# Bhumbra/probayes

Hardware: AMD Instinct MI355X
Metric: MH chain-steps/sec (whole node), 10-dim model, 65 536 chains, 1/2/4/8 GPU (higher is better)
Workload: dtype f64; 1 GPU; cfg2: 10-dim diagonal-Gaussian random-walk MH, 65536 chains/GPU, full trace every step; chains_per_gpu=65536, dim=10, trace=True, steps_per_launch=250, parallelism=chain-sharded x1

## Files before the change

probayes_amd/csrc/pbh_device.h:

```cpp
#pragma once
#include <hip/hip_runtime.h>
#include <stdint.h>

namespace pbh {

constexpr double kNearlyPosZero = 2.2250738585072014e-308;
constexpr double kNearlyPosInf = 1.7976931348623158e+308;
constexpr double kNearlyNegInf = -1.7976931348623158e+308;


struct u32x4 { uint32_t x, y, z, w; };

__device__ __forceinline__ u32x4 philox4x32_10(u32x4 c, uint32_t k0,
                                                uint32_t k1) {
  constexpr uint32_t M0 = 0xD2511F53u, M1 = 0xCD9E8D57u;
  constexpr uint32_t W0 = 0x9E3779B9u, W1 = 0xBB67AE85u;
#pragma unroll
  for (int i = 0; i < 10; ++i) {
    const uint64_t p0 = (uint64_t)M0 * c.x;
    const uint64_t p1 = (uint64_t)M1 * c.z;
    const uint32_t hi0 = (uint32_t)(p0 >> 32), lo0 = (uint32_t)p0;
    const uint32_t hi1 = (uint32_t)(p1 >> 32), lo1 = (uint32_t)p1;
    c = u32x4{(uint32_t)__builtin_amdgcn_bitop3_b32(hi1, c.y, k0, 0x96), lo1,
              (uint32_t)__builtin_amdgcn_bitop3_b32(hi0, c.w, k1, 0x96), lo0};
    k0 += W0;
    k1 += W1;
  }
  return c;
}

struct PhiloxKeys { uint32_t k0[10], k1[10]; };
__device__ __forceinline__ uint32_t in_vgpr(uint32_t v) {
  uint32_t r;
  asm("v_mov_b32 %0, %1" : "=v"(r) : "s"(v));
  return r;
}
__device__ __forceinline__ double in_vgpr_f64(double v) {
  const uint64_t b = __builtin_bit_cast(uint64_t, v);
  return __builtin_bit_cast(double, ((uint64_t)in_vgpr((uint32_t)(b >> 32)) << 32) |
                                        in_vgpr((uint32_t)b));
}
__device__ __forceinline__ PhiloxKeys philox_keys_v(uint32_t k0, uint32_t k1) {
  PhiloxKeys k;
#pragma unroll
  for (int i = 0; i < 10; ++i) {
    k.k0[i] = in_vgpr(k0 + (uint32_t)i * 0x9E3779B9u);
    k.k1[i] = in_vgpr(k1 + (uint32_t)i * 0xBB67AE85u);
  }
  return k;
}
__device__ __forceinline__ u32x4 philox4x32_10_rk(u32x4 c, const PhiloxKeys &k) {
  constexpr uint32_t M0 = 0xD2511F53u, M1 = 0xCD9E8D57u;
#pragma unroll
  for (int i = 0; i < 10; ++i) {
    const uint64_t p0 = (uint64_t)M0 * c.x;
    const uint64_t p1 = (uint64_t)M1 * c.z;
    const uint32_t hi0 = (uint32_t)(p0 >> 32), lo0 = (uint32_t)p0;
    const uint32_t hi1 = (uint32_t)(p1 >> 32), lo1 = (uint32_t)p1;
    c = u32x4{(uint32_t)__builtin_amdgcn_bitop3_b32(hi1, c.y, k.k0[i], 0x96), lo1,
              (uint32_t)__builtin_amdgcn_bitop3_b32(hi0, c.w, k.k1[i], 0x96), lo0};
  }
  return c;
}

struct Xo { uint32_t s0, s1, s2, s3; };

__device__ __forceinline__ uint32_t rotl32(uint32_t x, int k) {
  return (x << k) | (x >> (32 - k));
}

__device__ __forceinline__ uint32_t xo_next(Xo &s) {
  const uint32_t r = rotl32(s.s1 * 5u, 7) * 9u;
  const uint32_t t = s.s1 << 9;
  s.s2 ^= s.s0;
  s.s3 ^= s.s1;
  s.s1 ^= s.s2;
  s.s0 ^= s.s3;
  s.s2 ^= t;
  s.s3 = rotl32(s.s3, 11);
  return r;
}

__host__ __device__ __forceinline__ uint64_t splitmix64(uint64_t &z) {
  uint64_t x = (z += 0x9E3779B97F4A7C15ull);
  x = (x ^ (x >> 30)) * 0xBF58476D1CE4E5B9ull;
  x = (x ^ (x >> 27)) * 0x94D049BB133111EBull;
  return x ^ (x >> 31);
}

__device__ __forceinline__ double u01(uint32_t a, uint32_t b) {
  return ((double)(a >> 5) * 67108864.0 + (double)(b >> 6)) *
         (1.0 / 9007199254740992.0);
}

__device__ __forceinline__ void box_muller(u32x4 w, double &z0, double &z1) {
  const double u1 = 1.0 - u01(w.x, w.y);
  const double u2 = u01(w.z, w.w);
  const double r = sqrt(-2.0 * log(u1));
  double s, c;
  sincospi(2.0 * u2, &s, &c);
  z0 = r * c;
  z1 = r * s;
}

__device__ __forceinline__ double log_unit(double u) {
  const uint64_t b = __builtin_bit_cast(uint64_t, u);
  int e = (int)((b >> 52) & 0x7FF) - 1023;
  double m = __builtin_bit_cast(double, (b & 0x000FFFFFFFFFFFFFull) |
                                            0x3FF0000000000000ull);
  const bool big = m > 1.4142135623730951;
  m = big ? m * 0.5 : m;
  e += big ? 1 : 0;
  const double t = (m - 1.0) / (m + 1.0);
  const double s = t * t;
// ... 644 lines not shown
```

probayes_amd/csrc/pbh_engine.hip:

```cpp
#include <hip/hip_runtime.h>
#include <rccl/rccl.h>

#include <cmath>
#include <cstdarg>
#include <cstdio>
#include <cstdlib>
#include <cstring>
#include <string>
#include <algorithm>
#include <atomic>
#include <chrono>
#include <map>
#include <mutex>
#include <unordered_map>
#include <vector>

#include "../../include/pbhip.h"
#include "pbh_kernels.h"
#include "pbh_expr_host.h"
#include "pbh_device.h"

using pbh::KArgs;

struct pbh_engine {
// ... 1331 lines not shown
      return fail(PBH_ERR_STATE, "trace capacity %lld < %lld records",
                  (long long)e->cap, (long long)recs);
  }
  return PBH_OK;
}

static void run_args(pbh_engine *e, KArgs &k, size_t &lds) {
  k = e->k;
  k.n = e->n;
  k.off = e->off;
  k.x = e->x;
  k.lp = e->lp;
  k.rng = e->rng;
  k.seed_lo = (uint32_t)e->seed;
  k.seed_hi = (uint32_t)(e->seed >> 32);
  k.rep = e->rep;
#ifdef PBH_PHASES
  if (!k.rep) k.rep = phase_buffer();
#endif
  k.xo = e->xo;
  k.tx = e->tx; k.tlp = e->tlp; k.tpx = e->tpx; k.tpp = e->tpp; k.ts = e->ts;
  k.tacc = e->tacc;
  k.thin = e->cap > 0 ? e->thin : 1;
  k.rec_base = e->rec_base;
  k.rec_cap = e->cap;
  k.debug = e->debug;
  k.W = (e->n + 63) / 64;
  {
    const double v = k.tran_value;
    const double qt = k.pscale == PBH_PSCALE_LIN
                          ? v : (v <= k.log_npi ? std::exp(v) : 1.7976931348623158e+308);
    k.pair_ok = (e->pair_enabled && (k.scores == PBH_SCORES_METROPOLIS || qt > 0.0)) ? 1 : 0;
    k.simple_acc = (k.scores == PBH_SCORES_METROPOLIS ||
                    (k.scores == PBH_SCORES_HASTINGS &&
                     k.tran_kind == PBH_TRAN_CONST && qt > 0.0)) ? 1 : 0;
    k.acc_beta = (k.scores == PBH_SCORES_HASTINGS && !k.tran_sym) ? qt : 1.0;
  }
  k.gibbs_mfma = e->gibbs_mfma ? 1 : 0;
  k.gibbs_fast = e->gibbs_fast ? 1 : 0;
  k.gibbs_lanes = e->gibbs_lanes;
  k.gmm_lanes = e->gmm_lanes;
  k.gmm_full = e->gmm_full ? 1 : 0;
  k.pair_full = e->pair_full ? 1 : 0;
  k.iid_full = e->iid_full ? 1 : 0;
  k.fair = e->fair;
  k.pair_wg = e->pair_wg;
  k.gq = e->gq;
  k.moments = (e->collect & PBH_COLLECT_MOMENTS) ? 1 : 0;
  k.msum = e->msum; k.msq = e->msq; k.nacc = e->nacc;
  k.bm64 = e->bm64;
  lds = (k.target == PBH_TARGET_NORM_IID && k.tn <= 16384 &&
                      k.rng != PBH_RNG_PHILOX)
                         ? (size_t)k.tn * sizeof(double) : 0;
}

int pbh_run(pbh_engine *e, int64_t n_steps, int32_t steps_per_launch) {
  if (check_ptr(e, "engine")) return PBH_ERR_ARG;
  static const bool trace_enq = [] {
    const char *t = std::getenv("PBH_TRACE_ENQUEUE");
    return t && t[0] == '1';
  }();
  using clk = std::chrono::steady_clock;
  const auto tq0 = clk::now();
  auto tq = [&](const char *what) {
    if (trace_enq)
      std::fprintf(stderr, "pbh_run %s %.2f us\n", what,
                   std::chrono::duration<double, std::micro>(clk::now() - tq0).count());
  };
  if (const int rc = run_checks(e, n_steps)) return rc;
  if (n_steps == 0) {
    e->timed = false;
    e->last_launches = 0;
    return PBH_OK;
  }
  if (e->rng == PBH_RNG_REPLAY &&
      (!e->rep || e->g < e->rep_g0 || e->g + n_steps > e->rep_g0 + e->rep_steps))
    return fail(PBH_ERR_STATE,
                "replay stream covers steps [%lld, %lld), run needs [%lld, %lld)",
                (long long)e->rep_g0, (long long)(e->rep_g0 + e->rep_steps),
                (long long)e->g, (long long)(e->g + n_steps));
  if (e->srv_active && (steps_per_launch <= 0 || steps_per_launch >= n_steps) &&
      n_steps <= (1 << 30) && e->g + n_steps < (int64_t(1) << 47) &&
      !(e->collect & PBH_COLLECT_MOMENTS) && e->has_pred && e->cap > 0 && e->thin == 1 &&
      e->g - e->rec_base >= 0 && e->g + n_steps - e->rec_base <= e->cap) {
    if (e->srv_pending) {
      const int rc = srv_wait(e, e->srv_pending, false);
      e->srv_pending = 0;
      if (rc) return rc;
    }
    if (srv_clk::now() - e->srv_last <= std::chrono::milliseconds(e->srv_idle_ms / 2)) {
      const bool short_run = n_steps <= 64;
      srv_submit(e, n_steps, short_run ? e->fair_short : e->fair,
                 short_run ? 1 : e->fair_rel);
      tq("server command (fast path)");
      return PBH_OK;
    }
  }
  HIP_TRY(hipSetDevice(e->device));
  if (e->rng == PBH_RNG_XOSHIRO && !e->xo_seeded) {
    HIP_TRY(pbh::launch_xo_seed(e->xo, e->n, e->off, e->seed, e->stream));
    e->xo_seeded = true;
  }
  const int64_t spl = steps_per_launch > 0 ? steps_per_launch : n_steps;
  KArgs k;
  size_t lds = 0;
  run_args(e, k, lds);
  const bool gfast = e->has_gibbs && pbh::gibbs_fast_form(k);
  if (e->srv_enabled && !e->has_gibbs && spl >= n_steps && n_steps <= (1 << 30)) {
    pbh::KArgs kc = k;
    kc.g0 = e->g;
    kc.n_steps = (int32_t)n_steps;
    kc.has_pred = e->has_pred ? 1 : 0;
    const bool short_run = n_steps <= 64;
    kc.fair = short_run ? e->fair_short : e->fair;
    kc.fair_rel = short_run ? 1 : e->fair_rel;
    kc.srv_cmd = kc.srv_done = kc.srv_mail = reinterpret_cast<void *>(1);
    int32_t wgs = 0;
    const bool form = e->g + n_steps < (int64_t(1) << 47) &&
        (e->srv_active
             ? (!k.moments && e->has_pred && e->cap > 0 && e->thin == 1 &&
                e->g - e->rec_base >= 0 && e->g + n_steps - e->rec_base <= e->cap)
             : pbh::launch_mh_server(kc, e->stream, &wgs, true) == hipSuccess);
    if (form) {
      if (e->srv_active) {
        if (e->srv_pending) {
          const int rc = srv_wait(e, e->srv_pending, false);
          e->srv_pending = 0;
          if (rc) return rc;
        }
        const auto idle = srv_clk::now() - e->srv_last;
        if (idle > std::chrono::milliseconds(e->srv_idle_ms / 2) ||
            (idle > std::chrono::milliseconds(1) && srv_kernel_ended(e))) {
          const int rc = srv_stop(e);
          if (rc) return rc;
        }
      }
      if (!e->srv_active) {
        const int rc = srv_launch(e, kc);
        if (rc) return rc;
      }
      srv_submit(e, n_steps, kc.fair, kc.fair_rel);
      tq("server command");
      return PBH_OK;
    }
    (void)hipGetLastError();
  }
  SRV_STOP(e);
  e->srv_timed = false;
  pbh::LaunchEvents &lev = pbh::launch_events();
  tq("args");
  if (e->event_markers) {
    HIP_TRY(hipEventRecord(e->ev0, e->stream));
    tq("event0");
    lev = {};
  } else {
    lev.start = e->ev0;
    lev.stop = nullptr;
  }
  int64_t launches = 0;
  for (int64_t done = 0; done < n_steps;) {
    const int64_t m = std::min(spl, n_steps - done);
    if (!e->event_markers && done + m >= n_steps) lev.stop = e->ev1;
    k.n_steps = (int32_t)m;
    const bool short_launch = m <= 64;
    k.fair = short_launch ? e->fair_short : e->fair;
    k.fair_rel = short_launch ? 1 : e->fair_rel;
    k.g0 = e->g;
    k.has_pred = e->has_pred ? 1 : 0;
    k.rep_row0 = e->g - e->rep_g0;
    k.gq_init = e->gq_valid ? 0 : 1;
    k.lx = e->lx;
    k.lx_init = e->lx_valid ? 0 : 1;
    hipError_t err = e->has_gibbs ? pbh::launch_gibbs(k, e->stream)
                                  : pbh::launch_mh(k, e->stream, lds);
    if (err != hipSuccess) {
      lev = {};
      return fail(PBH_ERR_HIP, "kernel launch failed: %s", hipGetErrorString(err));
    }
    e->g += m;
    e->has_pred = true;
    e->gq_valid = gfast;
    e->lx_valid = !e->has_gibbs && k.ufun != 0 &&
                  (e->rng == PBH_RNG_PHILOX || e->rng == PBH_RNG_XOSHIRO);
    done += m;
    ++launches;
  }
  lev = {};
  tq("launches");
  if (e->event_markers) HIP_TRY(hipEventRecord(e->ev1, e->stream));
  tq("event1");
  e->mom_steps += n_steps;
  e->timed = true;
  e->last_launches = launches;
  return PBH_OK;
}

int pbh_legacy_run(pbh_engine *e, int64_t n_steps, int32_t steps_per_launch) {
  if (check_ptr(e, "engine")) return PBH_ERR_ARG;
  SRV_STOP(e);
  if (e->rng != PBH_RNG_REPLAY)
    return fail(PBH_ERR_STATE, "pbh_legacy_run runs the REPLAY RNG (pbh_set_rng)");
  if (!e->mt_key) return fail(PBH_ERR_STATE, "pbh_legacy_seed first");
  if (e->mt_stale)
    return fail(PBH_ERR_STATE, "pbh_restore ran after pbh_legacy_seed: set the "
// ... 1142 lines not shown
```

probayes_amd/csrc/pbh_kernels.h:

```cpp
#pragma once
#include <hip/hip_runtime.h>
#include <hip/hip_ext.h>
#include <stdint.h>

#include "pbh_expr_words.h"

namespace pbh {

struct LaunchEvents {
  hipEvent_t start = nullptr, stop = nullptr;
};
LaunchEvents &launch_events();
bool module_launch();
hipFunction_t kernel_function(const void *kernel);

template <typename F, typename... Args>
inline void pbh_launch(F kernel, const dim3 &grid, const dim3 &block,
                       size_t shm, hipStream_t st, Args... args) {
  LaunchEvents &ev = launch_events();
  if (ev.start || ev.stop) {
    (void)hipExtLaunchKernelGGL(kernel, grid, block, (uint32_t)shm, st, ev.start,
                                ev.stop, 0u, args...);
  } else if (const hipFunction_t fn = module_launch()
                 ? kernel_function(reinterpret_cast<const void *>(kernel)) : nullptr) {
// ... 39 lines not shown
  double norm_C;
  int64_t n;
  int64_t off;
  int32_t n_steps;
  int64_t g0;
  int32_t has_pred;
  double *x;
  double *lp;
  int32_t rng;
  uint32_t seed_lo, seed_hi;
  const double *rep;
  uint32_t *xo;
  int64_t rep_row0;
  int32_t R;
  double *tx, *tlp, *tpx, *tpp, *ts;
  uint64_t *tacc;
  int32_t thin;
  int64_t rec_base;
  int64_t rec_cap;
  int32_t debug;
  int64_t W;
  int32_t pair_ok;
  int32_t simple_acc;
  double acc_beta;
  int32_t gibbs_mfma;
  int32_t gibbs_fast;
  const double *gpp;
  const double *gmup;
  const double *gzlo, *gzhi;
  const double *gak;
  double gconst;
  double *gq;
  int32_t gq_init;
  double *lx;
  int32_t lx_init;
  int32_t gibbs_lanes;
  int32_t gmm_lanes;
  int32_t gmm_full;
  int32_t pair_full;
  int32_t iid_full;
  int32_t fair;
  int32_t pair_wg;
  int32_t fair_rel;
  void *srv_cmd;
  void *srv_done;
  void *srv_mail;
  int64_t srv_idle;
  int32_t srv_mode;
  int32_t moments;
  double *msum, *msq;
  int64_t *nacc;
  const double *bm64;
  const int32_t *ecode;
  const double *econst;
  int32_t en;
  const double *edata;
  const int32_t *eleaf;
  int32_t enobs, enpad, enleaf;
  int32_t ewide;
};
constexpr int kTargetExprData = 8;
struct alignas(16) SrvCmd {
  uint32_t seq, n;
  uint64_t arg;
};
__host__ __device__ inline uint64_t srv_arg(int64_t g0, uint32_t fair, uint32_t fair_rel,
                                            uint32_t op, uint32_t seq) {
  return ((uint64_t)g0 & 0xFFFFFFFFFFFFull) | ((uint64_t)(fair & 31u) << 48) |
         ((uint64_t)(fair_rel & 1u) << 53) | ((uint64_t)(op & 1u) << 54) |
         ((uint64_t)(seq & 0xFFu) << 56);
}
struct SrvDone {
  uint32_t seq, pad;
  uint64_t t0, t1;
  uint64_t pad2;
};
constexpr uint32_t kSrvRun = 0, kSrvExit = 1;


inline bool gibbs_fast_form(const KArgs &a) {
  return a.gibbs_fast && a.rng == 1  && !a.debug && a.d <= 16;
}

hipError_t launch_mh(const KArgs &a, hipStream_t s, size_t lds_bytes);
hipError_t launch_gibbs(const KArgs &a, hipStream_t s);
hipError_t launch_mh_server(const KArgs &a, hipStream_t s, int32_t *wgs, bool check);
hipError_t launch_xo_seed(uint32_t *xo, int64_t n, int64_t off, uint64_t seed,
                          hipStream_t s);
bool mh_dim_supported(int d);
hipError_t launch_mh_expr(const KArgs &a, hipStream_t s);
hipError_t launch_eval_expr(const KArgs &a, int64_t n, const double *x, double *out);
hipError_t launch_check_normals(int64_t n, const uint32_t *words, double *fast,
                                double *ref);
hipError_t launch_check_normals64(int64_t n, const uint32_t *words,
                                  const double *tab, double *fast, double *ref);
hipError_t launch_trace_stats(const double *tx, const uint64_t *tacc, int64_t n,
                              int32_t d, int64_t W, int64_t first,
                              int64_t count, double *sum, double *sumsq,
                              int64_t *nacc, hipStream_t s);
hipError_t launch_trace_expectation(const double *tx, const double *tlp,
                                    int64_t n, int32_t d, int64_t first,
                                    int64_t count, double exponent, int32_t lin,
                                    double log_npi, double *out, hipStream_t s);
hipError_t launch_trace_ess(const double *tx, int64_t n, int32_t d,
                            int64_t first, int64_t count, double *ess,
                            hipStream_t st, int fft, int32_t *list);
hipError_t launch_ess_total(const double *ess, int64_t n, int32_t d, double *total,
                            hipStream_t st);
void bm64_tables(double *out);
constexpr int kLegLogN = 129, kLegLogInv = 2 * kLegLogN, kLegLogDoubles = 3 * kLegLogN + 1;
void legacy_log_table(double *out);
struct LegacyArgs {
  uint32_t *key;
  int32_t *pos;
  double *gauss;
  int32_t *has_gauss;
  const int32_t *order;
  double *out;
  int64_t n, n_steps, step0;
  int32_t d, R, gibbs, normal;
  int32_t k4;
  int32_t vardelta;
  uint64_t vmode;
  const double *vdelta;
  const double *lgtab;
  int32_t wp;
  double *thr;
};
hipError_t launch_legacy_draws(const LegacyArgs &a, int32_t kind, double param,
                               hipStream_t s);
hipError_t launch_legacy_seed(uint32_t *key, int32_t *pos, double *gauss,
                              int32_t *has_gauss, const uint32_t *seeds,
                              int64_t n, bool k4, hipStream_t s);
hipError_t launch_legacy_gen(const LegacyArgs &a, hipStream_t s);
hipError_t launch_legacy_ahead(uint32_t *key, int32_t *pos, int64_t n, int32_t want,
                               hipStream_t s);
hipError_t launch_legacy_normalize(uint32_t *key, int32_t *pos, int64_t n, hipStream_t s);
hipError_t launch_legacy_mh(const LegacyArgs &la, const KArgs &a, hipStream_t s, bool check);

int bool_perm_max_cols();
int64_t bool_perm_scratch_words(int n_cu);
hipError_t launch_bool_perm_freq(const uint8_t *in, int64_t rows, int cols,
                                 unsigned long long *counts,
                                 unsigned long long *scratch, int n_cu,
                                 hipStream_t s);
hipError_t launch_check_accept(int64_t n, const double *lp, const double *lpp,
                               const uint32_t *t0, const uint32_t *t1,
                               int32_t lin, double log_npi, uint8_t *out);

struct LinregArgs {
  const double *x_obs, *y_obs;
  int64_t n_obs;
  double hyper[11], stats[5], bounds[6];
  double *state, *lp_state;
  const double *rand;
  double *tx, *tp;
  int64_t n, chain_offset, n_steps, step0;
  uint64_t seed;
  int32_t mode;
};
int64_t linreg_max_obs();
hipError_t launch_linreg_gibbs(const LinregArgs &a, hipStream_t s);

}
```

probayes_amd/csrc/pbh_kernels_impl.h:

```cpp
#pragma once
#include <utility>

#include "pbh_kernels.h"
#include "pbh_device.h"
#include "../../include/pbhip.h"

namespace pbh {

namespace {

constexpr int kBlock = 256;
constexpr int kPairFullBlock = 512;

__device__ __forceinline__ double cld(const double *p, int64_t i) {
  return ((const __attribute__((address_space(4))) double *)p)[i];
}

__device__ __forceinline__ double uni(double v) {
  const uint64_t u = __builtin_bit_cast(uint64_t, v);
  const uint32_t lo = __builtin_amdgcn_readfirstlane((uint32_t)u);
  const uint32_t hi = __builtin_amdgcn_readfirstlane((uint32_t)(u >> 32));
  return __builtin_bit_cast(double, (uint64_t)lo | ((uint64_t)hi << 32));
}

template <int D>
__device__ __forceinline__ void apply_tfun(const double *tf, double (&dl)[D]) {
  double out[D];
#pragma unroll
  for (int k = 0; k < D; ++k) {
    double acc = cld(tf, k * D) * dl[0];
#pragma unroll
    for (int j = 1; j < D; ++j) acc = acc + cld(tf, k * D + j) * dl[j];
    out[k] = acc;
  }
#pragma unroll
  for (int k = 0; k < D; ++k) dl[k] = out[k];
}

template <int D>
__device__ __forceinline__ constexpr int mvn_perm(int i) {
  return D <= 1 ? 0 : (D == 2 ? 1 - i : (i < D - 1 ? D - 2 - i : D - 1));
}

__device__ __forceinline__ double norm_logpdf(double x, double loc,
                                              double scale, double logscale,
                                              double logC) {
  const double y = (x - loc) / scale;
  return ((-(y * y)) / 2.0 - logC) - logscale;
}

__device__ __forceinline__ double norm_pdf(double x, double loc, double scale,
                                           double C) {
  const double y = (x - loc) / scale;
  return (exp((-(y * y)) / 2.0) / C) / scale;
}

__device__ __forceinline__ double uniform_pdf(double x, double lo,
                                              double scale) {
  const double y = (x - lo) / scale;
  return (0.0 <= y && y <= 1.0) ? 1.0 / scale : 0.0;
}

__device__ __forceinline__ Xo xo_load(const KArgs &a, int h, int64_t c) {
  return Xo{a.xo[(0 * 2 + h) * a.n + c], a.xo[(1 * 2 + h) * a.n + c],
            a.xo[(2 * 2 + h) * a.n + c], a.xo[(3 * 2 + h) * a.n + c]};
}

__device__ __forceinline__ void xo_store(const KArgs &a, int h, int64_t c,
                                         const Xo &s) {
  a.xo[(0 * 2 + h) * a.n + c] = s.s0;
  a.xo[(1 * 2 + h) * a.n + c] = s.s1;
  a.xo[(2 * 2 + h) * a.n + c] = s.s2;
  a.xo[(3 * 2 + h) * a.n + c] = s.s3;
}

__device__ __forceinline__ u32x4 ctr(uint32_t j, int64_t g, int64_t chain) {
  return u32x4{j, (uint32_t)g, (uint32_t)chain,
               (uint32_t)((uint64_t)chain >> 32) ^
                   ((uint32_t)((uint64_t)g >> 32) << 16)};
}

constexpr int kStepLead = 24;

template <int D>
__device__ __forceinline__ uint32_t step_draws(const KArgs &a, int64_t g,
                                               int64_t chain, const double *tab,
                                               double (&r)[D]) {
  constexpr int NP = (D + 1) / 2, NW = 3 * NP + 1, NB = (NW + 3) / 4;
  uint32_t w[4 * NB];
#pragma unroll
  for (int q = 0; q < NB; ++q) {
    const u32x4 b = philox4x32_10(ctr(q, g, chain), a.seed_lo, a.seed_hi);
    w[4 * q] = b.x;
    w[4 * q + 1] = b.y;
    w[4 * q + 2] = b.z;
    w[4 * q + 3] = b.w;
  }
#pragma unroll
  for (int p = 0; p < NP; ++p) {
    double z0, z1;
    bm96_pair(w[3 * p], w[3 * p + 1], w[3 * p + 2], tab, z0, z1);
    r[2 * p] = z0;
    if (2 * p + 1 < D) r[2 * p + 1] = z1;
  }
  return w[3 * NP] >> (32 - kStepLead);
}

template <int D>
__device__ __forceinline__ double mvn_density(const KArgs &a,
                                              const double (&x)[D]) {
  double dev[D];
#pragma unroll
  for (int i = 0; i < D; ++i) dev[i] = x[mvn_perm<D>(i)] - cld(a.ta, i);
  double sq[D];
#pragma unroll
  for (int j = 0; j < D; ++j) {
    double y = dev[0] * cld(a.tb, j);
#pragma unroll
    for (int i = 1; i < D; ++i) y = y + dev[i] * cld(a.tb, i * D + j);
    sq[j] = y * y;
  }
  const double maha = np_sum_regs<D>(sq, D);
  const double logpdf = -0.5 * (cld(a.tc, 0) + maha);
  return a.pscale == PBH_PSCALE_LIN ? exp(logpdf) : logpdf;
}

template <int D, int K>
__device__ __forceinline__ double gmm_fast(const KArgs &a, const double (&x)[D]) {
  double v[K];
#pragma unroll
  for (int k = 0; k < K; ++k) {
    const double w = cld(a.tw, k);
    double acc = cld(a.tw, K + k);
#pragma unroll
    for (int i = 0; i < D; ++i) {
      const double u = (x[i] - cld(a.tb, k * D + i)) * w;
      acc = __builtin_fma(-u, u, acc);
    }
    v[k] = acc;
  }
  double m = v[0];
#pragma unroll
  for (int k = 1; k < K; ++k) m = __builtin_fmax(m, v[k]);
  double sum = 0.;
#pragma unroll
  for (int k = 0; k < K; ++k) sum += fast_exp(v[k] - m);
  return m + log(sum);
}

template <int D, bool DATA>
__device__ __forceinline__ double expr_density(const KArgs &a, const double (&x)[D]);

template <int D, int TGT, bool FAST>
__device__ __forceinline__ double joint_density(const KArgs &a,
                                                const double (&x)[D],
                                                const double *obs_lds,
                                                bool use_lds,
                                                const double *lx = nullptr) {
  double out = 0.0;
  switch (TGT ? TGT : a.target) {
    case PBH_TARGET_DIAG_GAUSS: {
      if (FAST) {
// ... 974 lines not shown
            t = u01((t0 << (32 - PD::LB)) | (w.x >> PD::LB), w.y);
          } else {
            t = u01(t0, t1);
          }
          ex = ratio_accept(lpp, lp, t, lin, a.log_npi);
        }
        accm = (accm & ~needm) | (__ballot(ex) & needm);
      }
    }
    const uint64_t mhi = accm & kHi;
    const uint64_t macc = mhi | (mhi >> 32);
    const bool accl = __builtin_amdgcn_inverse_ballot_w64(macc);
#pragma unroll
    for (int i = 0; i < H; ++i) x[i] = sel_f64(macc, x[i], xp[i]);
    if (REPLAY) eB = sel_f64(macc, eB, eA);
    lp = sel_f64(macc, lp, lpp);
    if constexpr (mom) {
      nacc += accl ? 1 : 0;
#pragma unroll
      for (int i = 0; i < H; ++i) {
        ms[i] += x[i];
        mq[i] = __builtin_fma(x[i], x[i], mq[i]);
      }
    }
    const bool rec_now = ph == 0;
    const int64_t rec = ri;
    ph = (ph + 1 == a.thin) ? 0 : ph + 1;
    ri += (ph == 0) ? 1 : 0;
    if (rec_now && rec >= 0 && rec < a.rec_cap) {
      double *row = a.tx + rec * D * a.n;
      if (active) {
#pragma unroll
        for (int i = 0; i < H; ++i) st_buf(row, boff, i * bstride, x[i]);
        if (hi) st_buf(a.tlp + rec * a.n, loff, 0, lp);
      }
      if (lane == 32 && (c >> 5) < 2 * a.W)
        reinterpret_cast<uint32_t *>(a.tacc)[rec * 2 * a.W + (c >> 5)] =
            (uint32_t)((mhi & act_mask) >> 32);
    }
  };

  if constexpr (PHX) {
    double cA[H], cB[H];
    uint32_t ctA = 0, ctB = 0, t1 = 0;
    int s = 0;
    if constexpr (PD::F32) {
      double nA[H], nB[H];
      uint32_t ntA = 0, ntB = 0;
      PD::draw(a, s_bmt, h, a.g0 >> 1, chain, cA, cB, ctA, ctB);
      if ((a.g0 & 1) && s < a.n_steps) {
        step(s, cB, ctB, t1);
        ++s;
        if (s < a.n_steps)
          PD::draw(a, s_bmt, h, (a.g0 + s) >> 1, chain, cA, cB, ctA, ctB);
      }
      for (; s + 3 < a.n_steps; s += 4) {
        PD::draw(a, s_bmt, h, ((a.g0 + s) >> 1) + 1, chain, nA, nB, ntA, ntB);
        step(s, cA, ctA, t1);
        step(s + 1, cB, ctB, t1);
        PD::draw(a, s_bmt, h, ((a.g0 + s) >> 1) + 2, chain, cA, cB, ctA, ctB);
        step(s + 2, nA, ntA, t1);
        step(s + 3, nB, ntB, t1);
      }
      if (s + 1 < a.n_steps) {
        step(s, cA, ctA, t1);
        step(s + 1, cB, ctB, t1);
        s += 2;
        if (s < a.n_steps)
          PD::draw(a, s_bmt, h, (a.g0 + s) >> 1, chain, cA, cB, ctA, ctB);
      }
      if (s < a.n_steps) step(s, cA, ctA, t1);
    } else if constexpr (FULL) {
        int64_t g0v = a.g0;
        int32_t nsv = a.n_steps, fairv = a.fair, fair_relv = a.fair_rel;
        constexpr int NW = 3 * H + 1, NB = (NW + 3) / 4, QA = (H + 1) / 2;
        constexpr uint64_t kHi = 0xFFFFFFFF00000000ull;
        uint64_t inl = __ballot(__builtin_fabs(lp) <= 700.);
        const uint32_t lpoff = hi ? loff : kNoStore;
        const uint32_t lpbytes = (uint32_t)(a.n * 8);
        const uint32_t aoff = lane == 32 ? (uint32_t)((c >> 5) * 4) : kNoStore;
        const uint32_t abytes = (uint32_t)(a.W * 8);
        int64_t rec = g0v + s - a.rec_base;
        const PhiloxKeys rk = philox_keys_v(a.seed_lo, a.seed_hi);
        auto philox_from = [&](int64_t P, uint32_t (&w)[4 * NB], auto Q0) {
#pragma unroll
          for (int q = 0; q < 4 * decltype(Q0)::value; ++q) w[q] = 0u;
#pragma unroll
          for (int q = decltype(Q0)::value; q < NB; ++q) {
            const u32x4 b = philox4x32_10_rk(ctr(q + 16 * h, P, chain), rk);
            w[4 * q] = b.x;
            w[4 * q + 1] = b.y;
            w[4 * q + 2] = b.z;
            w[4 * q + 3] = b.w;
          }
        };
        auto philox = [&](int64_t P, uint32_t (&w)[4 * NB]) {
#pragma unroll
          for (int q = 0; q < NB; ++q) {
            const u32x4 b = philox4x32_10_rk(ctr(q + 16 * h, P, chain), rk);
            w[4 * q] = b.x;
            w[4 * q + 1] = b.y;
            w[4 * q + 2] = b.z;
            w[4 * q + 3] = b.w;
          }
        };
        auto normals = [&](const uint32_t (&w)[4 * NB], auto Q0, auto Q1,
                           double (&ra)[H], double (&rb)[H]) {
          constexpr int q0 = decltype(Q0)::value, q1 = decltype(Q1)::value;
#pragma unroll
          for (int q = q0; q < q1; ++q) {
            double z0, z1;
            bm96_pair(w[3 * q], w[3 * q + 1], w[3 * q + 2], s_bmt, z0, z1);
#pragma unroll
            for (int e = 0; e < 2; ++e) {
              const int n = 2 * q + e;
              const double z = e ? z1 : z0;
              if (n < H) ra[n] = z;
              else rb[n - H] = z;
            }
          }
        };
        auto step_full = [&](int si, const double (&r)[H], uint32_t t0) {
          double xp[H];
#pragma unroll
          for (int i = 0; i < H; ++i)
            xp[i] = LOC0 ? __builtin_fma(r[i], psc[i], x[i])
                         : x[i] + __builtin_fma(r[i], psc[i], plc[i]);
          double p0 = 0., p1 = 0.;
#pragma unroll
          for (int i = 0; i < H; ++i) {
            const double u = __builtin_fma(xp[i], cb[i], -ca[i]);
            if (i & 1) p1 = __builtin_fma(u, u, p1);
            else p0 = __builtin_fma(u, u, p0);
          }
          double lo, up;
          halves_f64(p0 + p1, lo, up);
          const double lpp = (-(lo + up)) - a.ksum;
          const float eL = __builtin_amdgcn_exp2f(
              (float)__builtin_fma(lpp - lp, 1.4426950408889634, 16.0));
          const float fl = (float)t0;
          const uint64_t inp = __ballot(__builtin_fabs(lpp) <= 700.);
          const uint64_t inr = inp & inl;
          const uint64_t af = __ballot(fl <= __builtin_fmaf(eL, 0.999996f, -1.0f));
          const uint64_t rf = __ballot(fl > eL * 1.000004f);
          uint64_t accm = inr & af;
          const uint64_t needm = ~(inr & (af | rf)) & kHi;
          if (needm) {
            bool ex = false;
            if (__builtin_amdgcn_inverse_ballot_w64(needm))
              ex = pair_exact(a.seed_lo, a.seed_hi, a.log_npi, g0v + si, chain, h,
                              t0, lpp, lp);
            accm = (accm & ~needm) | (__ballot(ex) & needm);
          }
          const uint64_t mhi = accm & kHi;
          const uint64_t macc = mhi | (mhi >> 32);
#pragma unroll
          for (int i = 0; i < H; ++i) x[i] = sel_f64(macc, x[i], xp[i]);
          lp = sel_f64(macc, lp, lpp);
          inl = (inl & ~macc) | (inp & macc);
          double *row = a.tx + rec * D * a.n;
#pragma unroll
          for (int i = 0; i < H; ++i) st_buf(row, boff, i * bstride, x[i]);
          st_buf_n(a.tlp + rec * a.n, lpbytes, lpoff, lp);
          st_buf32_n(reinterpret_cast<uint32_t *>(a.tacc + rec * a.W), abytes, aoff,
                     (uint32_t)(mhi >> 32));
          ++rec;
        };
        using I0 = std::integral_constant<int, 0>;
        using IA = std::integral_constant<int, QA>;
        using IH = std::integral_constant<int, H>;
        auto run_block = [&]() {
          if (g0v & 1) {
            constexpr int QB = 3 * (H / 2) / 4;
            uint32_t w[4 * NB];
            philox_from(g0v >> 1, w, std::integral_constant<int, QB>{});
            normals(w, std::integral_constant<int, H / 2>{}, IH{}, cA, cB);
            __builtin_amdgcn_s_waitcnt(0);
            step_full(0, cB, w[3 * H] & 0xFFFFu);
            s = 1;
          }
          if (s + 1 < nsv) {
            uint32_t w[4 * NB];
            philox((g0v + s) >> 1, w);
            normals(w, I0{}, IH{}, cA, cB);
            ctA = w[3 * H] >> 16;
            ctB = w[3 * H] & 0xFFFFu;
            if (s == 0) __builtin_amdgcn_s_waitcnt(0);
// ... 13 lines not shown
              step_full(s, cA, ctA);
              normals(nw, I0{}, IA{}, nA, nB);
              step_full(s + 1, cB, ctB);
              normals(nw, IA{}, IH{}, nA, nB);
  #pragma unroll
              for (int i = 0; i < H; ++i) {
                cA[i] = nA[i];
                cB[i] = nB[i];
              }
              ctA = nw[3 * H] >> 16;
              ctB = nw[3 * H] & 0xFFFFu;
            }
            step_full(s, cA, ctA);
            step_full(s + 1, cB, ctB);
            s += 2;
          }
          if (s < nsv) {
            uint32_t w[4 * NB];
            philox((g0v + s) >> 1, w);
            normals(w, I0{}, IA{}, cA, cB);
            if (s == 0) __builtin_amdgcn_s_waitcnt(0);
            step_full(s, cA, w[3 * H] >> 16);
          }
        };
        if constexpr (SRV) {
          __shared__ int64_t s_cmd[6];
          SrvCmd *const hcmd = reinterpret_cast<SrvCmd *>(a.srv_cmd);
          SrvCmd *const mail = reinterpret_cast<SrvCmd *>(a.srv_mail);
          SrvDone *const donep = reinterpret_cast<SrvDone *>(a.srv_done) + blockIdx.x;
          const bool poller = __builtin_amdgcn_readfirstlane((int)(threadIdx.x >> 6)) == 0;
          const bool direct = (a.srv_mode & 1) != 0;
          const bool relay = blockIdx.x == 0 && !direct;
          uint32_t seen = 0u;
          for (;;) {
            if (poller) {
              const uint64_t tw = __builtin_amdgcn_s_memrealtime();
              const SrvCmd *src = relay ? hcmd : mail;
              uint32_t q;
              u32x4v v;
              for (;;) {
                v = ld16_sys(src);
                q = (uint32_t)__builtin_amdgcn_readfirstlane((int)v.x);
                const uint32_t chk = (uint32_t)__builtin_amdgcn_readfirstlane((int)v.w) >> 24;
                if (q != seen && chk == (q & 0xFFu)) break;
                if (__builtin_amdgcn_s_memrealtime() - tw > (uint64_t)a.srv_idle) {
                  q = 0u;
                  break;
                }
                __builtin_amdgcn_s_sleep(1);
              }
              const uint64_t tsee = __builtin_amdgcn_s_memrealtime();
              if (relay && q) st16_sys(mail, v);
              const uint32_t n = (uint32_t)__builtin_amdgcn_readfirstlane((int)v.y);
              const uint64_t arg =
                  (uint64_t)(uint32_t)__builtin_amdgcn_readfirstlane((int)v.z) |
                  ((uint64_t)(uint32_t)__builtin_amdgcn_readfirstlane((int)v.w) << 32);
              const int64_t g0 = (int64_t)(arg & 0xFFFFFFFFFFFFull);
              const uint32_t fr = (uint32_t)(arg >> 48) & 31u, frel = (uint32_t)(arg >> 53) & 1u;
              const uint32_t op = (uint32_t)(arg >> 54) & 1u;
              s_cmd[0] = q;
              s_cmd[1] = op;
              s_cmd[2] = g0;
              s_cmd[3] = n;
              s_cmd[4] = ((int64_t)frel << 32) | fr;
              s_cmd[5] = (int64_t)tsee;
            }
            __syncthreads();
            const uint32_t q = (uint32_t)__builtin_amdgcn_readfirstlane((int)s_cmd[0]);
            const uint32_t op = (uint32_t)__builtin_amdgcn_readfirstlane((int)s_cmd[1]);
            if (q == 0u || op == kSrvExit) {
              if (poller && q != 0u)
                __hip_atomic_store(&donep->seq, q, __ATOMIC_RELAXED, __HIP_MEMORY_SCOPE_SYSTEM);
              break;
            }
            const int64_t c2 = s_cmd[2], c4 = s_cmd[4];
            g0v = (int64_t)(uint32_t)__builtin_amdgcn_readfirstlane((int)(uint32_t)c2) |
                  ((int64_t)__builtin_amdgcn_readfirstlane((int)(c2 >> 32)) << 32);
            nsv = __builtin_amdgcn_readfirstlane((int)s_cmd[3]);
            fairv = __builtin_amdgcn_readfirstlane((int)(uint32_t)c4);
            fair_relv = __builtin_amdgcn_readfirstlane((int)(c4 >> 32));
            const uint64_t tseen = (uint64_t)s_cmd[5];
            s = 0;
            rec = g0v - a.rec_base;
            run_block();
            __builtin_amdgcn_s_waitcnt(0);
            __syncthreads();
            if (poller) {
              __hip_atomic_store(&donep->t0, tseen, __ATOMIC_RELAXED, __HIP_MEMORY_SCOPE_SYSTEM);
              __hip_atomic_store(&donep->t1, (uint64_t)__builtin_amdgcn_s_memrealtime(),
                                 __ATOMIC_RELAXED, __HIP_MEMORY_SCOPE_SYSTEM);
              __builtin_amdgcn_s_waitcnt(0);
              __hip_atomic_store(&donep->seq, q, __ATOMIC_RELAXED, __HIP_MEMORY_SCOPE_SYSTEM);
            }
            seen = q;
          }
        } else {
          run_block();
        }
        PBH_PHASE(3);
    } else {
      if (a.g0 & 1) {
        PD::draw(a, s_bmt, h, a.g0 >> 1, chain, cA, cB, ctA, ctB);
        step(s, cB, ctB, t1);
        ++s;
      }
      for (; s + 1 < a.n_steps; s += 2) {
        PD::draw(a, s_bmt, h, (a.g0 + s) >> 1, chain, cA, cB, ctA, ctB);
        step(s, cA, ctA, t1);
        step(s + 1, cB, ctB, t1);
      }
      if (s < a.n_steps) {
        PD::draw(a, s_bmt, h, (a.g0 + s) >> 1, chain, cA, cB, ctA, ctB);
        step(s, cA, ctA, t1);
      }
    }
  } else {
    double r[H];
    uint32_t t0 = 0, t1 = 0;
    for (int s = 0; s < a.n_steps; ++s) step(s, r, t0, t1);
  }

  if (active) {
#pragma unroll
    for (int i = 0; i < H; ++i) a.x[(k0 + i) * a.n + c] = x[i];
    if (hi) a.lp[c] = lp;
    if constexpr (mom) {
#pragma unroll
      for (int i = 0; i < H; ++i) {
        a.msum[(k0 + i) * a.n + c] += ms[i];
        a.msq[(k0 + i) * a.n + c] += mq[i];
      }
      if (hi) a.nacc[c] += nacc;
    }
    if (RNG == PBH_RNG_XOSHIRO) xo_store(a, h, c, xs);
  }
  if constexpr (FULL) {
    PBH_PHASE(4);
    PBH_PHASE_STORE(a.rep, wave, lane);
  }
}
template <int L>
__device__ __forceinline__ void gather_f64(double v, double (&all)[L]) {
  if constexpr (L == 2) {
    halves_f64(v, all[0], all[1]);
  } else {
    static_assert(L == 4, "lanes per chain: 2 or 4");
    double ev, od;
    rowpair_f64(v, ev, od);
    halves_f64(ev, all[0], all[2]);
    halves_f64(od, all[1], all[3]);
  }
}

template <int L>
__device__ __forceinline__ void gather_u32(uint32_t v, uint32_t (&all)[L]) {
  if constexpr (L == 2) {
    const auto a = __builtin_amdgcn_permlane32_swap(v, v, false, false);
    all[0] = a[0];
    all[1] = a[1];
  } else {
    const auto r = __builtin_amdgcn_permlane16_swap(v, v, false, false);
    const auto e = __builtin_amdgcn_permlane32_swap(r[0], r[0], false, false);
    const auto o = __builtin_amdgcn_permlane32_swap(r[1], r[1], false, false);
    all[0] = e[0];
    all[2] = e[1];
    all[1] = o[0];
// ... 1097 lines not shown
  int cm = (int)(a.g0 % nblk) * ts;
  st.draw_cycle(a, a.g0 - a.g0 % nblk, chain);
  st.act = __ballot(st.active && p == 0);
  st.ph = (int)((a.g0 + 1) % a.thin);
  st.ri = (a.g0 + 1) / a.thin - 1 - a.rec_base;
  int64_t cyc = (a.g0 + nblk - 1) / nblk;

  uint32_t post_mask = 1u << (D - 1);
  for (int k = ts - 1; k < D; k += ts) post_mask |= 1u << k;
  __builtin_amdgcn_s_waitcnt(0);
  int s = 0;
  bool entry = true;
  bool have_next = false;
  while (s < a.n_steps) {
    if (cm == 0) {
      if (!entry) {
        if (have_next) {
#pragma unroll
          for (int ii = 0; ii < M; ++ii) st.zo[ii] = st.zn[ii];
          st.fix_trunc(a, a.g0 + s, chain);
        } else {
          st.draw_cycle(a, a.g0 + s, chain);
        }
      }
      if ((cyc & (kRefreshCycles - 1)) == 0) st.refresh(a);
      ++cyc;
    }
    entry = false;
    have_next = false;
    const int nst = min(nblk - cm / ts, a.n_steps - s);
    const int ke = min(D, cm + nst * ts);
    if (ts == 1 && cm == 0 && ke == D) {
      st.draw_raw(a, a.g0 + s + D, chain, st.zn);
      have_next = true;
      st.template cycle<true>(a, 0, D, post_mask, std::make_integer_sequence<int, D>{});
    } else
      st.template cycle<false>(a, cm, ke, post_mask, std::make_integer_sequence<int, D>{});
    s += nst;
    cm = ke == D ? 0 : ke;
  }
  st.lp = st.vprob(a, st.Q);
  if (st.active) {
    const int64_t c = st.c;
#pragma unroll
    for (int ii = 0; ii < M; ++ii) {
      a.x[(p * M + ii) * a.n + c] = st.xo[ii];
      if (a.moments) {
        a.msum[(p * M + ii) * a.n + c] += st.ms[ii];
        a.msq[(p * M + ii) * a.n + c] += st.mq[ii];
      }
      a.gq[(p * M + ii) * a.n + c] = st.go[ii];
    }
    if (p == 0) {
      a.lp[c] = st.lp;
      if (a.moments) a.nacc[c] += a.n_steps;
      a.gq[D * a.n + c] = st.Q;
    }
  }
}

}

template <int D, int TGT, int PROP>
void launch_mh_spec(const KArgs &a, hipStream_t st, size_t lds) {
  const dim3 grid((unsigned)((a.n + kBlock - 1) / kBlock)), block(kBlock);
  if (a.rng == PBH_RNG_REPLAY)
    pbh_launch((mh_kernel<D, PBH_RNG_REPLAY, TGT, PROP>), grid, block,
                       lds, st, a);
  else if (a.rng == PBH_RNG_PHILOX)
    pbh_launch((mh_kernel<D, PBH_RNG_PHILOX, TGT, PROP>), grid, block,
                       lds, st, a);
  else if (a.rng == PBH_RNG_XOSHIRO)
    pbh_launch((mh_kernel<D, PBH_RNG_XOSHIRO, TGT, PROP>), grid, block,
                       lds, st, a);
  else
    pbh_launch((mh_kernel<D, PBH_RNG_PHILOX_F64, TGT, PROP>), grid,
                       block, lds, st, a);
}

inline bool pair_full_form(const KArgs &a) {
  return a.pair_full && a.rng == PBH_RNG_PHILOX && a.has_pred && a.thin == 1 &&
         a.pscale != PBH_PSCALE_LIN && a.tx != nullptr && a.n % 32 == 0 &&
         a.n * 8 <= (int64_t)kNoStore &&
         a.g0 - a.rec_base >= 0 && a.g0 + a.n_steps - a.rec_base <= a.rec_cap;
}

inline bool iid_full_form(const KArgs &a) {
  return a.iid_full && a.rng == PBH_RNG_PHILOX && a.simple_acc && !a.debug &&
         a.has_pred && a.thin == 1 && a.pscale != PBH_PSCALE_LIN && a.tx != nullptr &&
         !a.has_tfun && a.vint == 0 && a.bnd_on == 0 && !a.moments &&
         a.ufun < (1u << a.d) && a.n * 8 <= (int64_t)kNoStore &&
         (int64_t)a.n_steps * a.d * a.n * 8 <= (int64_t)kNoStore &&
         a.g0 - a.rec_base >= 0 && a.g0 + a.n_steps - a.rec_base <= a.rec_cap;
}

template <int D, bool MOM>
void launch_mh_pair_m(const KArgs &a, hipStream_t st, dim3 grid, dim3 block) {
  if constexpr (!MOM) {
    if (pair_full_form(a)) {
      if (a.ploc_zero)
        pbh_launch((mh_pair_kernel<D, PBH_RNG_PHILOX, false, true, true>), grid, block, 0, st, a);
      else
        pbh_launch((mh_pair_kernel<D, PBH_RNG_PHILOX, false, false, true>), grid, block, 0, st, a);
      return;
    }
  }
  if (a.rng == PBH_RNG_REPLAY)
    pbh_launch((mh_pair_kernel<D, PBH_RNG_REPLAY, MOM>), grid, block, 0, st, a);
  else if (a.rng == PBH_RNG_PHILOX && a.ploc_zero)
    pbh_launch((mh_pair_kernel<D, PBH_RNG_PHILOX, MOM, true>), grid, block, 0, st, a);
  else if (a.rng == PBH_RNG_PHILOX)
    pbh_launch((mh_pair_kernel<D, PBH_RNG_PHILOX, MOM>), grid, block, 0, st, a);
  else if (a.rng == PBH_RNG_XOSHIRO)
    pbh_launch((mh_pair_kernel<D, PBH_RNG_XOSHIRO, MOM>), grid, block, 0, st, a);
  else if (a.rng == PBH_RNG_PHILOX_FP32)
    pbh_launch((mh_pair_kernel<D, PBH_RNG_PHILOX_FP32, MOM>), grid, block, 0, st, a);
  else
    pbh_launch((mh_pair_kernel<D, PBH_RNG_PHILOX_F64, MOM>), grid, block, 0, st, a);
}

template <int D>
void launch_mh_pair(const KArgs &a, hipStream_t st) {
  const int64_t waves = (a.n + 31) / 32;
  if (!a.moments && pair_full_form(a)) {
    const int wg = a.pair_wg == kPairFullBlock ? kPairFullBlock : kBlock;
    const dim3 grid((unsigned)((waves * 64 + wg - 1) / wg)), block(wg);
    launch_mh_pair_m<D, false>(a, st, grid, block);
    return;
  }
  const dim3 grid((unsigned)((waves * 64 + kBlock - 1) / kBlock)), block(kBlock);
  if (a.moments) launch_mh_pair_m<D, true>(a, st, grid, block);
  else launch_mh_pair_m<D, false>(a, st, grid, block);
}

inline bool pair_form(const KArgs &a);
template <int D>
hipError_t launch_mh_server_d(const KArgs &a, hipStream_t st, int32_t *wgs, bool check) {
  if constexpr (D % 2 == 0 && D >= 4) {
    if (!(pair_form(a) && a.pair_ok && !a.moments && pair_full_form(a) &&
          a.pair_wg == kPairFullBlock && a.srv_cmd && a.srv_done && a.srv_mail))
      return hipErrorNotSupported;
    const int64_t waves = a.n / 32;
    const int64_t grid = (waves * 64 + kPairFullBlock - 1) / kPairFullBlock;
    const void *kern = a.ploc_zero
        ? reinterpret_cast<const void *>(mh_pair_kernel<D, PBH_RNG_PHILOX, false, true, true, true>)
        : reinterpret_cast<const void *>(mh_pair_kernel<D, PBH_RNG_PHILOX, false, false, true, true>);
    int dev = 0, cus = 0, per = 0;
    hipError_t err = hipGetDevice(&dev);
    if (err == hipSuccess) err = hipDeviceGetAttribute(&cus, hipDeviceAttributeMultiprocessorCount, dev);
    if (err == hipSuccess)
      err = hipOccupancyMaxActiveBlocksPerMultiprocessor(&per, kern, kPairFullBlock, 0);
    if (err != hipSuccess) return err;
    if ((int64_t)per * cus < grid) return hipErrorNotSupported;
    if (wgs) *wgs = (int32_t)grid;
    if (check) return hipSuccess;
    if (a.ploc_zero)
      hipLaunchKernelGGL((mh_pair_kernel<D, PBH_RNG_PHILOX, false, true, true, true>),
                         dim3((unsigned)grid), dim3(kPairFullBlock), 0, st, a);
    else
      hipLaunchKernelGGL((mh_pair_kernel<D, PBH_RNG_PHILOX, false, false, true, true>),
                         dim3((unsigned)grid), dim3(kPairFullBlock), 0, st, a);
    return hipGetLastError();
  } else {
    (void)a; (void)st; (void)wgs; (void)check;
    return hipErrorNotSupported;
  }
}
// ... 184 lines not shown
```

Baseline: 46.94 billion chain-steps/s.

## Precompute step-invariant Philox rounds per chain and reuse across steps

Adds a Philox prefix structure that precomputes the parts of the first rounds depending only on block index, chain and high step bits. Each step then only computes the step-dependent remainder from round 2 onward, saving several multiplies per block. The prefix is rebuilt when the high step bits change, and the fast paths are guarded so a run does not cross a 2^33 step boundary. This costs extra registers to hold the prefix per block.

```diff
diff --git a/probayes_amd/csrc/pbh_device.h b/probayes_amd/csrc/pbh_device.h
--- a/probayes_amd/csrc/pbh_device.h
+++ b/probayes_amd/csrc/pbh_device.h
@@ -2,14 +2,14 @@
 #include <hip/hip_runtime.h>
 #include <stdint.h>
 
+#include "pbh_philox.h"
+
 namespace pbh {
 
 constexpr double kNearlyPosZero = 2.2250738585072014e-308;
 constexpr double kNearlyPosInf = 1.7976931348623158e+308;
 constexpr double kNearlyNegInf = -1.7976931348623158e+308;
 
-
-struct u32x4 { uint32_t x, y, z, w; };
 
 __device__ __forceinline__ u32x4 philox4x32_10(u32x4 c, uint32_t k0,
                                                 uint32_t k1) {
@@ -29,7 +29,6 @@
   return c;
 }
 
-struct PhiloxKeys { uint32_t k0[10], k1[10]; };
 __device__ __forceinline__ uint32_t in_vgpr(uint32_t v) {
   uint32_t r;
   asm("v_mov_b32 %0, %1" : "=v"(r) : "s"(v));
diff --git a/probayes_amd/csrc/pbh_engine.hip b/probayes_amd/csrc/pbh_engine.hip
--- a/probayes_amd/csrc/pbh_engine.hip
+++ b/probayes_amd/csrc/pbh_engine.hip
@@ -1437,7 +1437,8 @@
   if (e->srv_active && (steps_per_launch <= 0 || steps_per_launch >= n_steps) &&
       n_steps <= (1 << 30) && e->g + n_steps < (int64_t(1) << 47) &&
       !(e->collect & PBH_COLLECT_MOMENTS) && e->has_pred && e->cap > 0 && e->thin == 1 &&
-      e->g - e->rec_base >= 0 && e->g + n_steps - e->rec_base <= e->cap) {
+      e->g - e->rec_base >= 0 && e->g + n_steps - e->rec_base <= e->cap &&
+      pbh::pair_index_hi_const(e->g, n_steps)) {
     if (e->srv_pending) {
       const int rc = srv_wait(e, e->srv_pending, false);
       e->srv_pending = 0;
@@ -1474,7 +1475,8 @@
     const bool form = e->g + n_steps < (int64_t(1) << 47) &&
         (e->srv_active
              ? (!k.moments && e->has_pred && e->cap > 0 && e->thin == 1 &&
-                e->g - e->rec_base >= 0 && e->g + n_steps - e->rec_base <= e->cap)
+                e->g - e->rec_base >= 0 && e->g + n_steps - e->rec_base <= e->cap &&
+                pbh::pair_index_hi_const(e->g, n_steps))
              : pbh::launch_mh_server(kc, e->stream, &wgs, true) == hipSuccess);
     if (form) {
       if (e->srv_active) {
diff --git a/probayes_amd/csrc/pbh_kernels.h b/probayes_amd/csrc/pbh_kernels.h
--- a/probayes_amd/csrc/pbh_kernels.h
+++ b/probayes_amd/csrc/pbh_kernels.h
@@ -145,6 +145,10 @@
   return a.gibbs_fast && a.rng == 1  && !a.debug && a.d <= 16;
 }
 
+inline bool pair_index_hi_const(int64_t g0, int64_t n) {
+  return n < 1 || (g0 >> 33) == ((g0 + n - 1) >> 33);
+}
+
 hipError_t launch_mh(const KArgs &a, hipStream_t s, size_t lds_bytes);
 hipError_t launch_gibbs(const KArgs &a, hipStream_t s);
 hipError_t launch_mh_server(const KArgs &a, hipStream_t s, int32_t *wgs, bool check);
diff --git a/probayes_amd/csrc/pbh_kernels_impl.h b/probayes_amd/csrc/pbh_kernels_impl.h
--- a/probayes_amd/csrc/pbh_kernels_impl.h
+++ b/probayes_amd/csrc/pbh_kernels_impl.h
@@ -75,9 +75,7 @@
 }
 
 __device__ __forceinline__ u32x4 ctr(uint32_t j, int64_t g, int64_t chain) {
-  return u32x4{j, (uint32_t)g, (uint32_t)chain,
-               (uint32_t)((uint64_t)chain >> 32) ^
-                   ((uint32_t)((uint64_t)g >> 32) << 16)};
+  return philox_ctr(j, g, chain);
 }
 
 constexpr int kStepLead = 24;
@@ -1218,27 +1216,14 @@
         const uint32_t abytes = (uint32_t)(a.W * 8);
         int64_t rec = g0v + s - a.rec_base;
         const PhiloxKeys rk = philox_keys_v(a.seed_lo, a.seed_hi);
+        uint32_t pre_hi = (uint32_t)((uint64_t)g0v >> 33);
+        PhiloxPrefix<NB> pre =
+            philox_prefix<NB>(16u * (uint32_t)h, chain, pre_hi, a.seed_lo, a.seed_hi);
         auto philox_from = [&](int64_t P, uint32_t (&w)[4 * NB], auto Q0) {
-#pragma unroll
-          for (int q = 0; q < 4 * decltype(Q0)::value; ++q) w[q] = 0u;
-#pragma unroll
-          for (int q = decltype(Q0)::value; q < NB; ++q) {
-            const u32x4 b = philox4x32_10_rk(ctr(q + 16 * h, P, chain), rk);
-            w[4 * q] = b.x;
-            w[4 * q + 1] = b.y;
-            w[4 * q + 2] = b.z;
-            w[4 * q + 3] = b.w;
-          }
+          philox_prefix_blocks<NB, decltype(Q0)::value>((uint32_t)P, pre, rk, w);
         };
         auto philox = [&](int64_t P, uint32_t (&w)[4 * NB]) {
-#pragma unroll
-          for (int q = 0; q < NB; ++q) {
-            const u32x4 b = philox4x32_10_rk(ctr(q + 16 * h, P, chain), rk);
-            w[4 * q] = b.x;
-            w[4 * q + 1] = b.y;
-            w[4 * q + 2] = b.z;
-            w[4 * q + 3] = b.w;
-          }
+          philox_prefix_blocks<NB>((uint32_t)P, pre, rk, w);
         };
         auto normals = [&](const uint32_t (&w)[4 * NB], auto Q0, auto Q1,
                            double (&ra)[H], double (&rb)[H]) {
@@ -1418,6 +1403,10 @@
             const uint64_t tseen = (uint64_t)s_cmd[5];
             s = 0;
             rec = g0v - a.rec_base;
+            if ((uint32_t)((uint64_t)g0v >> 33) != pre_hi) {
+              pre_hi = (uint32_t)((uint64_t)g0v >> 33);
+              pre = philox_prefix<NB>(16u * (uint32_t)h, chain, pre_hi, a.seed_lo, a.seed_hi);
+            }
             run_block();
             __builtin_amdgcn_s_waitcnt(0);
             __syncthreads();
@@ -2681,7 +2670,8 @@
   return a.pair_full && a.rng == PBH_RNG_PHILOX && a.has_pred && a.thin == 1 &&
          a.pscale != PBH_PSCALE_LIN && a.tx != nullptr && a.n % 32 == 0 &&
          a.n * 8 <= (int64_t)kNoStore &&
-         a.g0 - a.rec_base >= 0 && a.g0 + a.n_steps - a.rec_base <= a.rec_cap;
+         a.g0 - a.rec_base >= 0 && a.g0 + a.n_steps - a.rec_base <= a.rec_cap &&
+         pair_index_hi_const(a.g0, a.n_steps);
 }
 
 inline bool iid_full_form(const KArgs &a) {
diff --git a/probayes_amd/csrc/pbh_philox.h b/probayes_amd/csrc/pbh_philox.h
--- /dev/null
+++ b/probayes_amd/csrc/pbh_philox.h
@@ -0,0 +1,94 @@
+#pragma once
+#include <stdint.h>
+
+#if defined(__HIPCC__)
+#define PBH_PHILOX_FN __host__ __device__ __forceinline__
+#else
+#define PBH_PHILOX_FN inline
+#endif
+#if defined(__clang__)
+#define PBH_UNROLL _Pragma("unroll")
+#else
+#define PBH_UNROLL
+#endif
+
+namespace pbh {
+
+struct u32x4 { uint32_t x, y, z, w; };
+
+constexpr uint32_t kPhiloxM0 = 0xD2511F53u, kPhiloxM1 = 0xCD9E8D57u;
+constexpr uint32_t kPhiloxW0 = 0x9E3779B9u, kPhiloxW1 = 0xBB67AE85u;
+
+PBH_PHILOX_FN uint32_t xor3(uint32_t a, uint32_t b, uint32_t c) {
+#if defined(__HIP_DEVICE_COMPILE__)
+  return (uint32_t)__builtin_amdgcn_bitop3_b32(a, b, c, 0x96);
+#else
+  return a ^ b ^ c;
+#endif
+}
+
+PBH_PHILOX_FN u32x4 philox_ctr(uint32_t j, int64_t g, int64_t chain) {
+  return u32x4{j, (uint32_t)g, (uint32_t)chain,
+               (uint32_t)((uint64_t)chain >> 32) ^
+                   ((uint32_t)((uint64_t)g >> 32) << 16)};
+}
+
+struct PhiloxKeys { uint32_t k0[10], k1[10]; };
+
+template <int NB>
+struct PhiloxPrefix {
+  uint32_t a;
+  uint32_t b[NB], c[NB], d[NB], e[NB];
+};
+
+template <int NB>
+PBH_PHILOX_FN PhiloxPrefix<NB> philox_prefix(uint32_t j0, int64_t chain, uint32_t g_hi,
+                                      uint32_t seed_lo, uint32_t seed_hi) {
+  const u32x4 c0 = philox_ctr(j0, (int64_t)((uint64_t)g_hi << 32), chain);
+  const uint64_t pc = (uint64_t)kPhiloxM1 * c0.z;
+  const uint32_t y1 = (uint32_t)pc;
+  PhiloxPrefix<NB> p;
+  p.a = (uint32_t)(pc >> 32) ^ seed_lo;
+PBH_UNROLL
+  for (int q = 0; q < NB; ++q) {
+    const uint64_t pj = (uint64_t)kPhiloxM0 * (j0 + (uint32_t)q);
+    const uint32_t z1 = (uint32_t)(pj >> 32) ^ c0.w ^ seed_hi;
+    const uint64_t pz = (uint64_t)kPhiloxM1 * z1;
+    const uint32_t x2 = (uint32_t)(pz >> 32) ^ y1 ^ (seed_lo + kPhiloxW0);
+    const uint64_t px = (uint64_t)kPhiloxM0 * x2;
+    p.b[q] = (uint32_t)pj ^ (seed_hi + kPhiloxW1);
+    p.c[q] = (uint32_t)pz ^ (seed_lo + 2u * kPhiloxW0);
+    p.d[q] = (uint32_t)(px >> 32) ^ (seed_hi + 2u * kPhiloxW1);
+    p.e[q] = (uint32_t)px;
+  }
+  return p;
+}
+
+template <int NB, int Q0 = 0>
+PBH_PHILOX_FN void philox_prefix_blocks(uint32_t g_lo, const PhiloxPrefix<NB> &p,
+                                 const PhiloxKeys &k, uint32_t (&w)[4 * NB]) {
+  const uint32_t x1 = p.a ^ g_lo;
+  const uint64_t p1 = (uint64_t)kPhiloxM0 * x1;
+  const uint32_t hi1 = (uint32_t)(p1 >> 32), w2 = (uint32_t)p1;
+PBH_UNROLL
+  for (int q = 0; q < 4 * Q0; ++q) w[q] = 0u;
+PBH_UNROLL
+  for (int q = Q0; q < NB; ++q) {
+    const uint32_t z2 = hi1 ^ p.b[q];
+    const uint64_t p2 = (uint64_t)kPhiloxM1 * z2;
+    u32x4 c{(uint32_t)(p2 >> 32) ^ p.c[q], (uint32_t)p2, w2 ^ p.d[q], p.e[q]};
+PBH_UNROLL
+    for (int i = 3; i < 10; ++i) {
+      const uint64_t m0 = (uint64_t)kPhiloxM0 * c.x;
+      const uint64_t m1 = (uint64_t)kPhiloxM1 * c.z;
+      c = u32x4{xor3((uint32_t)(m1 >> 32), c.y, k.k0[i]), (uint32_t)m1,
+                xor3((uint32_t)(m0 >> 32), c.w, k.k1[i]), (uint32_t)m0};
+    }
+    w[4 * q] = c.x;
+    w[4 * q + 1] = c.y;
+    w[4 * q + 2] = c.z;
+    w[4 * q + 3] = c.w;
+  }
+}
+
+}
```

Measured after the change: 48.69 billion chain-steps/s, median of 6. 3.7% higher.
